# MiloszKrajewski/K4os.Compression.LZ4

Measured on NVIDIA H100. Metric: GB/s uncompressed (encode+decode) on batched 64KiB blocks @1/2/4/8 GPU vs CPU ref, higher is better.
Workload: dtype u8

## Files before the change

### k4os/compression/lz4_b200/csrc/encode_chain.cuh

```cuda
#pragma once
#include "common.cuh"
#include "encode_generic.cuh"
#include "encode_tile.cuh"

namespace k4 {

struct ChainState {
    uint32_t table[4096];
    uint32_t currentOffset;
    uint32_t dictSize;
    uint32_t reserved[2];
};
static_assert(sizeof(ChainState) == 16400, "K4LZ4_CHAIN_STATE_BYTES");

#ifndef K4_ENC_CHAIN_WARPS
#define K4_ENC_CHAIN_WARPS 32
#endif
constexpr int ENC_CHAIN_WARPS = K4_ENC_CHAIN_WARPS;

__device__ int encode_chain_warp(const uint8_t* __restrict__ src, const uint32_t n, const uint32_t P,
                                 uint8_t* __restrict__ dst, const int cap, ChainState* st) {
    const int lane = lane_id();
    uint32_t* const table = st->table;
    uint32_t startIndex = __ldcg(&st->currentOffset), dsz = __ldcg(&st->dictSize);
    if (startIndex + n > 0x80000000u) {
        const uint32_t delta = startIndex - 65536u;
        for (int i = lane; i < 4096; i += 32) {
            const uint32_t t = __ldcg(table + i);
            __stcg(table + i, t < delta ? 0u : t - delta);
        }
        startIndex = 65536u;
        if (dsz > 65536u) dsz = 65536u;
    }
    if (n > (uint32_t)MAX_INPUT_SIZE) {
        if (lane == 0) { __stcg(&st->currentOffset, startIndex); __stcg(&st->dictSize, dsz); }
        __syncwarp();
        return 0;
    }
    const uint32_t d = dsz < P ? dsz : P;
    const bool dictSmall = d < 65536u && d < startIndex;
    const uint32_t prefixIdxLimit = startIndex - d;
    if (lane == 0) { __stcg(&st->currentOffset, startIndex + n); __stcg(&st->dictSize, d + n); }
    auto accept = [&](uint32_t idx, uint32_t cur) {
        return idx < cur && !(dictSmall && idx < prefixIdxLimit) && !(idx + (uint32_t)MAX_DISTANCE < cur);
    };
#define RD32(p) ldg_u32u(src + (int)(p))
#define RD8(p) ((uint32_t)__ldg(src + (int)(p)))
#define HASH(p) hash5(ldg_u64u(src + (p)), 12)
    const int64_t olimit = cap;
    uint32_t ip = 0, anchor = 0, op = 0;

    if (n >= (uint32_t)MINLENGTH) {
        const uint32_t mfl1 = n - MFLIMIT + 1, mlim = n - LASTLITERALS;
        if (lane == 0) __stcg(table + HASH(0), startIndex);
        __syncwarp();
        ip = 1;
        bool post = false;
        uint32_t q0 = 0;
        uint32_t base = 1;
        for (;;) {
            uint32_t h2 = 0xFFFFFFFFu;
            if (post) h2 = HASH(ip - 2);
            const bool isPost = post && lane == 0;
            const uint32_t q = q0 + (uint32_t)lane - (post ? 1u : 0u);
            const uint32_t pos = isPost ? ip : base + probe_advance(q);
            const bool valid = isPost || (base + probe_advance(q + 1) <= mfl1);
            const uint64_t v64 = valid ? ldg_u64u(src + pos) : 0ull;
            const uint32_t v = (uint32_t)v64;
            const uint32_t h = valid ? hash5(v64, 12) : (0x10000u + (uint32_t)lane);
            uint32_t cand = valid ? __ldcg(table + h) : 0u;
            if (h == h2) cand = startIndex + ip - 2;
            const unsigned peers = __match_any_sync(FULL, h);
            const unsigned earlier = peers & ((1u << lane) - 1u);
            const int fromLane = earlier ? 31 - __clz(earlier) : lane;
            const uint32_t fwdPos = __shfl_sync(FULL, pos, fromLane);
            if (earlier) cand = startIndex + fwdPos;
            const uint32_t cur = startIndex + pos;
            bool hit = false;
            if (valid && accept(cand, cur)) hit = RD32(cand - startIndex) == v;
            const unsigned hits = __ballot_sync(FULL, hit);
            const unsigned ends = __ballot_sync(FULL, !valid);
            const int f = hits ? __ffs(hits) - 1 : 32;
            const int e = ends ? __ffs(ends) - 1 : 32;
            {
                const int last = e < f ? e - 1 : f;
                const unsigned upto = (last >= 31) ? 0xffffffffu : ((1u << (last + 1)) - 1u);
                const unsigned later = peers & ~((2u << lane) - 1u) & upto;
                const bool doStore = valid && ((1u << lane) & upto) && !(lane < 31 ? later : 0u);
                if (post) {
                    const unsigned same2 = __ballot_sync(FULL, valid && h == h2) & upto;
                    if (lane == 0 && !same2) __stcg(table + h2, startIndex + ip - 2);
                }
                if (doStore) __stcg(table + h, cur);
                __syncwarp();
            }
            if (e < f) break;
            if (f == 32) {
                if (post) { post = false; base = ip + 1; q0 = 31; }
                else q0 += 32;
                continue;
            }
            const bool zeroLit = post && f == 0;
            int m = (int)(__shfl_sync(FULL, cand, f) - startIndex);
            ip = __shfl_sync(FULL, pos, f);
            const uint32_t a0h = ip + MINMATCH;
            const int b0h = m + MINMATCH;
            uint32_t x1 = 0u;
            {
                const uint32_t a = a0h + 4u * lane;
                if (lane < 8 && (int)mlim - (int)a > 0) x1 = RD32(a) ^ RD32(b0h + 4 * lane);
            }
            uint32_t caught = 0;
            if (!zeroLit) {
                for (int width = 8;; width = 32) {
                    const bool part = lane < width;
                    const bool ok = !part || ((ip > anchor + lane) && (m - lane > -(int)d) &&
                                              (RD8(ip - 1 - lane) == RD8(m - 1 - lane)));
                    const unsigned bad = __ballot_sync(FULL, !ok);
                    const int c = bad ? __ffs(bad) - 1 : width;
                    ip -= c; m -= c; caught += (uint32_t)c;
                    if (bad) break;
                }
            }
            const uint32_t lit = ip - anchor;
            if (!zeroLit && (int64_t)op + 1 + lit + 8 + lit / 255 > olimit) return 0;
            uint32_t mc = caught;
            {
                uint32_t a0 = a0h;
                int b0 = b0h;
                for (int width = 8;; width = 32) {
                    const uint32_t a = a0 + 4u * lane;
                    const int bb = b0 + 4 * lane;
                    const bool part = lane < width;
                    const int room = (int)mlim - (int)a;
                    const uint32_t x = width == 8 ? x1 : ((part && room > 0) ? (RD32(a) ^ RD32(bb)) : 0u);
                    int eq = x ? ((__ffs(x) - 1) >> 3) : 4;
                    if (eq > room) eq = room < 0 ? 0 : room;
                    if (!part) eq = 4;
                    const unsigned stop = __ballot_sync(FULL, eq < 4);
                    if (stop) {
                        const int s = __ffs(stop) - 1;
                        mc += 4u * s + (uint32_t)__shfl_sync(FULL, eq, s);
                        break;
                    }
                    mc += 4u * width; a0 += 4u * width; b0 += 4 * width;
                }
            }
            const uint32_t hdr = run_header_size(lit);
            const uint32_t afterOff = op + hdr + lit + 2;
            if ((int64_t)afterOff + 6 + (mc + 240) / 255 > olimit) return 0;
            {
                const uint32_t mlTok = mc >= 15 ? 15u : mc;
                const uint32_t off = (uint32_t)((int)ip - m);
                if (lane == 0) {
                    if (lit >= 15) {
                        uint32_t o = op, rest = lit - 15;
                        dst[o++] = (uint8_t)(0xF0 | mlTok);
                        for (; rest >= 255; rest -= 255) dst[o++] = 255;
                        dst[o] = (uint8_t)rest;
                    } else dst[op] = (uint8_t)((lit << 4) | mlTok);
                    dst[afterOff - 2] = (uint8_t)off;
                    dst[afterOff - 1] = (uint8_t)(off >> 8);
                }
                for (uint32_t i = lane; i < lit; i += 32) dst[op + hdr + i] = (uint8_t)RD8(anchor + i);
                op = afterOff;
                if (mc >= 15) {
                    const uint32_t rest = mc - 15, nff = rest / 255;
                    for (uint32_t i = lane; i < nff; i += 32) dst[op + i] = 0xFF;
                    if (lane == 0) dst[op + nff] = (uint8_t)(rest % 255);
                    op += nff + 1;
                }
            }
            ip += mc + MINMATCH;
            anchor = ip;
            if (ip >= mfl1) break;
            post = true; q0 = 0; base = ip + 1;
        }
    }
    {
        const uint32_t run = n - anchor;
        if ((int64_t)op + run + 1 + (run + 255 - 15) / 255 > olimit) return 0;
        const uint32_t hdr = run_header_size(run);
        if (lane == 0) write_run_header(dst, op, run);
        op += hdr;
        for (uint32_t i = lane; i < run; i += 32) dst[op + i] = (uint8_t)RD8(anchor + i);
        op += run;
        return (int)op;
    }
#undef RD32
#undef RD8
#undef HASH
}

__global__ void __launch_bounds__(32, ENC_CHAIN_WARPS)
encode_chain_kernel(const uint8_t* __restrict__ srcBase, const int64_t* __restrict__ srcOff,
                    const int32_t* __restrict__ srcLen, const int32_t* __restrict__ prefixLen,
                    uint8_t* __restrict__ dstBase, const int64_t* __restrict__ dstOff,
                    const int32_t* __restrict__ dstCap, uint8_t* __restrict__ stateBase,
                    const int64_t* __restrict__ stateOff, int32_t* __restrict__ outLen, int nBlocks, int level,
                    uint32_t* __restrict__ nextBlock) {
    const int lane = lane_id();
    for (;;) {
        int b = 0;
        if (lane == 0) b = (int)atomicAdd(nextBlock, 1u);
        b = __shfl_sync(FULL, b, 0);
        if (b >= nBlocks) return;
        const int n = srcLen[b];
        if (n <= 0) { if (lane == 0) outLen[b] = 0; continue; }
        if (level >= 3) { if (lane == 0) outLen[b] = -2; continue; }
        const int P = prefixLen[b];
        uint8_t* const sp = stateBase + stateOff[b];
        if (P < 0 || (reinterpret_cast<uintptr_t>(sp) & 15)) { if (lane == 0) outLen[b] = -1; continue; }
        const int r = encode_chain_warp(srcBase + srcOff[b], (uint32_t)n, (uint32_t)P, dstBase + dstOff[b],
                                        dstCap[b], reinterpret_cast<ChainState*>(sp));
        if (lane == 0) {
            outLen[b] = r <= 0 ? -1 : r;
            atomicAdd(&g_encode_stats[3], 1ull);
        }
        __syncwarp();
    }
}

}
```

### k4os/compression/lz4_b200/csrc/encode_tile.cuh

```cuda
#pragma once
#include "common.cuh"
#include "encode_generic.cuh"

namespace k4 {


__device__ __forceinline__ uint32_t lds_u32u(const uint8_t* p) {
    const uintptr_t a = reinterpret_cast<uintptr_t>(p);
    const uint32_t* w = reinterpret_cast<const uint32_t*>(a & ~uintptr_t(3));
    return __funnelshift_r(w[0], w[1], (uint32_t)(a & 3) * 8);
}

#ifndef K4_ENC_OVL
#define K4_ENC_OVL 1
#endif
#ifndef K4_ENC_PF
#define K4_ENC_PF 0
#endif
#ifndef K4_ENC_WIN
#define K4_ENC_WIN 16
#endif
#ifndef K4_ENC_SPEC
#define K4_ENC_SPEC 1
#endif
static_assert(K4_ENC_WIN >= 0 && K4_ENC_WIN <= 32, "K4_ENC_WIN: lanes of a run's first batch, 1..32 (0 = 32)");
__device__ __forceinline__ void prefetch_l1(const void* p) { asm volatile("prefetch.global.L1 [%0];" :: "l"(p)); }

__device__ __forceinline__ uint32_t probe_advance(uint32_t q) {
    if (q <= 64u) return q;
    if (q == 0) return 0;
    const uint32_t c = 63u + q, k = c >> 6;
    return 1u + 32u * k * (k - 1u) + (c - 64u * k) * k;
}

template <bool STAGED, bool HARD = true, bool GTAB = false, int TAGMODE = (K4_ENC_TAGS ? 1 : 0), int WIN = 32>
__device__ int encode_spec_warp(const uint8_t* __restrict__ src, const uint8_t* sin, const uint32_t n,
                                uint8_t* __restrict__ dst, const int cap, const int hardCap, uint16_t* table) {
    const int lane = lane_id();
    const int64_t hard = hardCap;
#define RD32(p) (STAGED ? lds_u32u(sin + (p)) : ldg_u32u(src + (p)))
#ifndef K4_ENC_GTAB_L1
#define K4_ENC_GTAB_L1 0
#endif
#define TGET(h) ((GTAB && !K4_ENC_GTAB_L1) ? (uint32_t)__ldcg(table + (h)) : (uint32_t)table[(h)])
    constexpr bool TAGS = TAGMODE != 0;
    constexpr uint32_t TAG_SHIFT = TAGMODE == 2 ? 3u : 11u, TAG_MASK = TAGMODE == 2 ? 0xFFFFu : 0xFFu;
    uint8_t* const tags = reinterpret_cast<uint8_t*>(table) + ENC_TABLE_BYTES;
    uint32_t* const table32 = reinterpret_cast<uint32_t*>(table);
    auto tagGet = [&](uint32_t h) -> uint32_t {
        return (GTAB && !K4_ENC_GTAB_L1) ? (uint32_t)__ldcg(tags + h) : (uint32_t)tags[h];
    };
    auto slotPut = [&](uint32_t h, uint32_t pos, uint32_t tg) {
        if (TAGMODE == 2) {
            if (GTAB) __stcg(table32 + h, pos | (tg << 16)); else table32[h] = pos | (tg << 16);
        } else {
            if (GTAB && !K4_ENC_GTAB_L1) __stcg(table + h, (uint16_t)pos); else table[h] = (uint16_t)pos;
            if (TAGS) { if (GTAB && !K4_ENC_GTAB_L1) __stcg(tags + h, (uint8_t)tg); else tags[h] = (uint8_t)tg; }
        }
    };
#define RD8(p) (STAGED ? (uint32_t)sin[(p)] : (uint32_t)__ldg(src + (p)))
    {
        const uint32_t t0 = (TAGS && n >= 4) ? (((RD32(0) * 2654435761u) >> TAG_SHIFT) & TAG_MASK) : 0u;
        const uint32_t fillT = TAGMODE == 2 ? (t0 << 16) : 0u;
        uint4* t = reinterpret_cast<uint4*>(table);
        constexpr int TBYTES = TAGMODE == 2 ? 2 * ENC_TABLE_BYTES : ENC_TABLE_BYTES;
        for (int i = lane; i < TBYTES / 16; i += 32) {
            if (GTAB) __stcg(t + i, make_uint4(fillT, fillT, fillT, fillT)); else t[i] = make_uint4(fillT, fillT, fillT, fillT);
        }
        if (TAGMODE == 1 || TAGMODE == 3) {
            const uint32_t b4 = t0 * 0x01010101u;
            uint4* g = reinterpret_cast<uint4*>(tags);
            for (int i = lane; i < (ENC_TABLE_BYTES / 2) / 16; i += 32) {
                if (GTAB) __stcg(g + i, make_uint4(b4, b4, b4, b4)); else g[i] = make_uint4(b4, b4, b4, b4);
            }
        }
        __syncwarp();
    }
    const bool limited = !(cap >= max_output_size((int)n));
    const int64_t olimit = cap;
    uint32_t ip = 0, anchor = 0, op = 0;

    if (n >= (uint32_t)MINLENGTH) {
        const uint32_t mfl1 = n - MFLIMIT + 1, mlim = n - LASTLITERALS;
        if (lane == 0) { const uint32_t p0 = RD32(0) * 2654435761u; slotPut(p0 >> 19, 0u, (p0 >> TAG_SHIFT) & TAG_MASK); }
        __syncwarp();
        ip = 1;
        bool post = false;
        uint32_t q0 = 0;
        uint32_t base = 1;
        constexpr uint32_t WIN0 = (WIN <= 0 || WIN > 32) ? 32u : (uint32_t)WIN;
        constexpr bool NARROW = WIN0 < 32u;
        uint32_t width = WIN0;
        for (;;) {
            uint32_t h2 = 0xFFFFFFFFu, tag2 = 0;
            if (post) { const uint32_t p2 = RD32(ip - 2) * 2654435761u; h2 = p2 >> 19; tag2 = (p2 >> TAG_SHIFT) & TAG_MASK; }
            const bool isPost = post && lane == 0;
            const uint32_t q = q0 + (uint32_t)lane - (post ? 1u : 0u);
            const uint32_t pos = isPost ? ip : base + probe_advance(q);
            const bool inWin = !NARROW || (uint32_t)lane < width;
            const bool valid = inWin && (isPost || (base + probe_advance(q + 1) <= mfl1));
            const uint32_t v = valid ? RD32(pos) : 0u;
            const uint32_t prod = v * 2654435761u;
            const uint32_t h = valid ? prod >> 19 : (0x10000u + (uint32_t)lane);
            const uint32_t tg = (prod >> TAG_SHIFT) & TAG_MASK;
            uint32_t cand = 0u, ctag = tg;
            bool lazyPos = false;
            if (TAGMODE == 2) {
                const uint32_t e32 = valid ? ((GTAB && !K4_ENC_GTAB_L1) ? __ldcg(table32 + h) : table32[h]) : 0xFFFF0000u;
                cand = e32 & 0xFFFFu; ctag = e32 >> 16;
                if (!valid) ctag = 0x10000u;
            } else if (TAGMODE == 3) {
                ctag = valid ? tagGet(h) : 0x100u;
                lazyPos = true;
            } else {
                cand = valid ? TGET(h) : 0u;
                if (TAGMODE == 1) ctag = valid ? tagGet(h) : 0x100u;
            }
            if (h == h2) { cand = ip - 2; ctag = TAGS ? tag2 : tg; lazyPos = false; }
            const unsigned peers = __match_any_sync(FULL, h);
            const unsigned earlier = peers & ((1u << lane) - 1u);
            const int fromLane = earlier ? 31 - __clz(earlier) : lane;
            const uint32_t fwdPos = __shfl_sync(FULL, pos, fromLane);
            const uint32_t fwdTag = __shfl_sync(FULL, tg, fromLane);
            if (earlier) { cand = fwdPos; ctag = TAGS ? fwdTag : tg; lazyPos = false; }
            constexpr bool SPEC = K4_ENC_SPEC && TAGMODE == 2 && K4_ENC_OVL;
            bool hit = false;
            if (!SPEC && valid && ctag == tg) {
                if (TAGMODE == 3 && lazyPos) cand = TGET(h);
                hit = RD32(cand) == v;
                if (TAGS && !STAGED && (K4_ENC_PF & 1)) {
                    prefetch_l1(src + (cand + 32u < n ? cand + 32u : n - 1u));
                    if (cand >= 8u) prefetch_l1(src + cand - 8u);
                }
            }
            if (!STAGED && (K4_ENC_PF & 2) && lane == 0) prefetch_l1(src + (pos + 384u < n ? pos + 384u : n - 1u));
            const unsigned ends = __ballot_sync(FULL, inWin && !valid);
            const int e = ends ? __ffs(ends) - 1 : 32;
            int f = 32;
            uint32_t sm = 0u, sip = 0u, sx1 = 0u;
            bool sok = true;
            if (SPEC) {
                for (unsigned agree = __ballot_sync(FULL, valid && ctag == tg); agree; agree &= agree - 1u) {
                    const int c = __ffs(agree) - 1;
                    if (e < c) break;
                    sm = __shfl_sync(FULL, cand, c);
                    sip = __shfl_sync(FULL, pos, c);
                    const uint32_t vc = __shfl_sync(FULL, v, c);
                    bool same = true;
                    sx1 = 0u; sok = true;
                    if (lane < 8) {
                        const uint32_t a = sip + MINMATCH + 4u * lane;
                        if ((int)mlim - (int)a > 0) sx1 = RD32(a) ^ RD32(sm + MINMATCH + 4u * lane);
                        sok = (sip > anchor + lane) && (sm > (uint32_t)lane) && (RD8(sip - 1 - lane) == RD8(sm - 1 - lane));
                    } else if (lane == 8) {
                        same = RD32(sm) == vc;
                    }
                    if (__all_sync(FULL, same)) { f = c; break; }
                }
            } else {
                const unsigned hits = __ballot_sync(FULL, hit);
                f = hits ? __ffs(hits) - 1 : 32;
            }
            if (e < f) break;
            {
                const unsigned upto = (f >= 31) ? 0xffffffffu : ((2u << f) - 1u);
                const unsigned later = peers & ~((2u << lane) - 1u) & upto;
                const bool doStore = valid && ((1u << lane) & upto) && !(lane < 31 ? later : 0u);
                if (post) {
                    const unsigned same2 = __ballot_sync(FULL, valid && h == h2) & upto;
                    if (lane == 0 && !same2) {
                        slotPut(h2, ip - 2, tag2);
                    }
                }
                if (doStore) slotPut(h, pos, tg);
                __syncwarp();
            }
            if (f == 32) {
                const uint32_t w = NARROW ? width : 32u;
                if (post) { post = false; base = ip + 1; q0 = w - 1; }
                else q0 += w;
                width = 32;
                continue;
            }
            const bool zeroLit = post && f == 0;
            uint32_t m = SPEC ? sm : __shfl_sync(FULL, cand, f);
            ip = SPEC ? sip : __shfl_sync(FULL, pos, f);
            const uint32_t a0h = ip + MINMATCH, b0h = m + MINMATCH;
            uint32_t x1 = sx1;
            if (K4_ENC_OVL && !SPEC) {
                const uint32_t a = a0h + 4u * lane;
                if (lane < 8 && (int)mlim - (int)a > 0) x1 = RD32(a) ^ RD32(b0h + 4u * lane);
            }
            uint32_t caught = 0;
            if (!zeroLit) {
                for (int width = 8;; width = 32) {
                    const bool part = lane < width;
                    const bool ok = (SPEC && width == 8) ? sok
                                  : (!part || ((ip > anchor + lane) && (m > (uint32_t)lane) &&
                                               (RD8(ip - 1 - lane) == RD8(m - 1 - lane))));
                    const unsigned bad = __ballot_sync(FULL, !ok);
                    const int c = bad ? __ffs(bad) - 1 : width;
                    ip -= c; m -= c; caught += (uint32_t)c;
                    if (bad) break;
                }
            }
            const uint32_t lit = ip - anchor;
            if (!zeroLit && limited && (int64_t)op + 1 + lit + 8 + lit / 255 > olimit) return 0;
            uint32_t mc = caught;
            {
                uint32_t a0 = a0h, b0 = b0h;
                for (int width = 8;; width = 32) {
                    const uint32_t a = a0 + 4u * lane, bb = b0 + 4u * lane;
                    const bool part = lane < width;
                    const int room = (int)mlim - (int)a;
                    const uint32_t x = (K4_ENC_OVL && width == 8) ? x1 : ((part && room > 0) ? (RD32(a) ^ RD32(bb)) : 0u);
                    int eq = x ? ((__ffs(x) - 1) >> 3) : 4;
                    if (eq > room) eq = room < 0 ? 0 : room;
                    if (!part) eq = 4;
                    const unsigned stop = __ballot_sync(FULL, eq < 4);
                    if (stop) {
                        const int s = __ffs(stop) - 1;
                        mc += 4u * s + (uint32_t)__shfl_sync(FULL, eq, s);
                        break;
                    }
                    mc += 4u * width; a0 += 4u * width; b0 += 4u * width;
                }
            }
            const uint32_t hdr = run_header_size(lit);
            const uint32_t afterOff = op + hdr + lit + 2;
            if (limited && (int64_t)afterOff + 6 + (mc + 240) / 255 > olimit) return 0;
            if (HARD && (int64_t)afterOff + (mc >= 15 ? (mc - 15) / 255 + 1 : 0) > hard) return 0;
            {
                const uint32_t mlTok = mc >= 15 ? 15u : mc;
                if (lane == 0) {
                    if (lit >= 15) {
                        uint32_t o = op, rest = lit - 15;
                        dst[o++] = (uint8_t)(0xF0 | mlTok);
                        for (; rest >= 255; rest -= 255) dst[o++] = 255;
                        dst[o] = (uint8_t)rest;
                    } else dst[op] = (uint8_t)((lit << 4) | mlTok);
                    dst[afterOff - 2] = (uint8_t)(ip - m);
                    dst[afterOff - 1] = (uint8_t)((ip - m) >> 8);
                }
                for (uint32_t i = lane; i < lit; i += 32) dst[op + hdr + i] = RD8(anchor + i);
                op = afterOff;
                if (mc >= 15) {
                    const uint32_t rest = mc - 15, nff = rest / 255;
                    for (uint32_t i = lane; i < nff; i += 32) dst[op + i] = 0xFF;
                    if (lane == 0) dst[op + nff] = (uint8_t)(rest % 255);
                    op += nff + 1;
                }
            }
            ip += mc + MINMATCH;
            anchor = ip;
            if (ip >= mfl1) break;
            post = true; q0 = 0; base = ip + 1; width = WIN0;
        }
    }
    {
        const uint32_t run = n - anchor;
        if (limited && (int64_t)op + run + 1 + (run + 255 - 15) / 255 > olimit) return 0;
        const uint32_t hdr = run_header_size(run);
        if (HARD && (int64_t)op + hdr + run > hard) return 0;
        if (lane == 0) write_run_header(dst, op, run);
        op += hdr;
        for (uint32_t i = lane; i < run; i += 32) dst[op + i] = RD8(anchor + i);
        op += run;
        return (int)op;
    }
#undef RD32
#undef TGET
#undef RD8
}

__device__ unsigned long long g_encode_stats[4];

template <bool GTAB>
__device__ __forceinline__ void encode_persistent_warp(
        const uint8_t* __restrict__ srcBase, const int64_t* __restrict__ srcOff,
        const int32_t* __restrict__ srcLen, uint8_t* __restrict__ dstBase,
        const int64_t* __restrict__ dstOff, const int32_t* __restrict__ dstCap,
        int32_t* __restrict__ outLen, const int nBlocks, int level,
        uint32_t* __restrict__ nextBlock, uint16_t* const table, const int reserve) {
    const int lane = lane_id();
    const bool enforce32 = (level & ENC_FLAG_X32) != 0;
    level &= 0xFF;
    for (;;) {
        int b = 0;
        if (lane == 0) {
            if (GTAB && (int)*(volatile uint32_t*)nextBlock >= nBlocks - reserve) b = nBlocks;
            else b = (int)atomicAdd(nextBlock, 1u);
        }
        b = __shfl_sync(FULL, b, 0);
        if (b >= nBlocks) return;
        const int n_ = srcLen[b];
        const uint8_t* __restrict__ src = srcBase + srcOff[b];
        uint8_t* __restrict__ dst = dstBase + dstOff[b];
        const int cap = dstCap[b];
        if (n_ <= 0) { if (lane == 0) outLen[b] = 0; continue; }
        if (level >= 3) { if (lane == 0) outLen[b] = -2; continue; }
        int r;
        if (n_ >= LIMIT_64K) r = encode_block_warp(src, n_, dst, cap, 0x7fffffff, table, enforce32);
        else r = encode_spec_warp<false, false, GTAB, GTAB ? ENC_GTAG : (K4_ENC_TAGS ? 1 : 0), K4_ENC_WIN>(src, nullptr, (uint32_t)n_, dst, cap, 0x7fffffff, table);
        if (lane == 0) {
            outLen[b] = r <= 0 ? -1 : r;
            atomicAdd(&g_encode_stats[n_ >= LIMIT_64K ? 2 : (GTAB ? 1 : 0)], 1ull);
        }
        __syncwarp();
    }
}

__global__ void __launch_bounds__(32)
encode_spec_kernel(const uint8_t* __restrict__ srcBase, const int64_t* __restrict__ srcOff,
                   const int32_t* __restrict__ srcLen, uint8_t* __restrict__ dstBase,
                   const int64_t* __restrict__ dstOff, const int32_t* __restrict__ dstCap,
                   int32_t* __restrict__ outLen, int nBlocks, int level, uint32_t* __restrict__ nextBlock) {
    extern __shared__ __align__(128) uint8_t smem_encs[];
    encode_persistent_warp<false>(srcBase, srcOff, srcLen, dstBase, dstOff, dstCap, outLen, nBlocks, level,
                                  nextBlock, reinterpret_cast<uint16_t*>(smem_encs), 0);
}

__global__ void __launch_bounds__(32)
encode_spec_gtab_kernel(const uint8_t* __restrict__ srcBase, const int64_t* __restrict__ srcOff,
                        const int32_t* __restrict__ srcLen, uint8_t* __restrict__ dstBase,
                        const int64_t* __restrict__ dstOff, const int32_t* __restrict__ dstCap,
                        int32_t* __restrict__ outLen, int nBlocks, int level, uint32_t* __restrict__ nextBlock,
                        uint8_t* __restrict__ gtab, int reserve) {
    encode_persistent_warp<true>(srcBase, srcOff, srcLen, dstBase, dstOff, dstCap, outLen, nBlocks, level, nextBlock,
                                 reinterpret_cast<uint16_t*>(gtab + (size_t)blockIdx.x * ENC_GSLOT_BYTES), reserve);
}

}
```

Baseline: 51.62.

## Batch LZ4 sequence emission per warp with lane-parallel scan-based writes

Instead of writing each sequence's token, literals, offset and match-length bytes as soon as it is found (lane 0 writes headers, the warp copies literals), the encoder records up to 32 sequences, one per lane, and flushes them together. The flush uses a warp prefix sum to compute output offsets, so each lane writes its own sequence and copies short literals with word loads, while long literal runs are copied cooperatively by the whole warp. This removes serial per-sequence store work from the match-finding loop, at the cost of extra registers, divergent per-lane byte stores and deferred writes whose error and early-return paths must stay consistent.

After: 52.48 (median of 6 runs). 1.7% higher.

```diff
diff --git a/k4os/compression/lz4_b200/csrc/encode_chain.cuh b/k4os/compression/lz4_b200/csrc/encode_chain.cuh
--- a/k4os/compression/lz4_b200/csrc/encode_chain.cuh
+++ b/k4os/compression/lz4_b200/csrc/encode_chain.cuh
@@ -49,6 +49,7 @@
 #define HASH(p) hash5(ldg_u64u(src + (p)), 12)
     const int64_t olimit = cap;
     uint32_t ip = 0, anchor = 0, op = 0;
+    SeqGroup grp;
 
     if (n >= (uint32_t)MINLENGTH) {
         const uint32_t mfl1 = n - MFLIMIT + 1, mlim = n - LASTLITERALS;
@@ -149,30 +150,11 @@
             const uint32_t hdr = run_header_size(lit);
             const uint32_t afterOff = op + hdr + lit + 2;
             if ((int64_t)afterOff + 6 + (mc + 240) / 255 > olimit) return 0;
-            {
-                const uint32_t mlTok = mc >= 15 ? 15u : mc;
-                const uint32_t off = (uint32_t)((int)ip - m);
-                if (lane == 0) {
-                    if (lit >= 15) {
-                        uint32_t o = op, rest = lit - 15;
-                        dst[o++] = (uint8_t)(0xF0 | mlTok);
-                        for (; rest >= 255; rest -= 255) dst[o++] = 255;
-                        dst[o] = (uint8_t)rest;
-                    } else dst[op] = (uint8_t)((lit << 4) | mlTok);
-                    dst[afterOff - 2] = (uint8_t)off;
-                    dst[afterOff - 1] = (uint8_t)(off >> 8);
-                }
-                for (uint32_t i = lane; i < lit; i += 32) dst[op + hdr + i] = (uint8_t)RD8(anchor + i);
-                op = afterOff;
-                if (mc >= 15) {
-                    const uint32_t rest = mc - 15, nff = rest / 255;
-                    for (uint32_t i = lane; i < nff; i += 32) dst[op + i] = 0xFF;
-                    if (lane == 0) dst[op + nff] = (uint8_t)(rest % 255);
-                    op += nff + 1;
-                }
-            }
+            seq_record(grp, ip, mc, (uint32_t)((int)ip - m));
+            op = afterOff + (mc >= 15 ? (mc - 15) / 255 + 1 : 0);
             ip += mc + MINMATCH;
             anchor = ip;
+            if (grp.n == 32) seq_flush(grp, src, dst, anchor, op);
             if (ip >= mfl1) break;
             post = true; q0 = 0; base = ip + 1;
         }
@@ -181,6 +163,7 @@
         const uint32_t run = n - anchor;
         if ((int64_t)op + run + 1 + (run + 255 - 15) / 255 > olimit) return 0;
         const uint32_t hdr = run_header_size(run);
+        if (grp.n) seq_flush(grp, src, dst, anchor, op);
         if (lane == 0) write_run_header(dst, op, run);
         op += hdr;
         for (uint32_t i = lane; i < run; i += 32) dst[op + i] = (uint8_t)RD8(anchor + i);
diff --git a/k4os/compression/lz4_b200/csrc/encode_tile.cuh b/k4os/compression/lz4_b200/csrc/encode_tile.cuh
--- a/k4os/compression/lz4_b200/csrc/encode_tile.cuh
+++ b/k4os/compression/lz4_b200/csrc/encode_tile.cuh
@@ -31,6 +31,75 @@
     if (q == 0) return 0;
     const uint32_t c = 63u + q, k = c >> 6;
     return 1u + 32u * k * (k - 1u) + (c - 64u * k) * k;
+}
+
+struct SeqGroup {
+    uint32_t ip = 0, mc = 0, off = 0;
+    uint32_t anchor = 0, op = 0;
+    int n = 0;
+};
+
+__device__ __forceinline__ void seq_record(SeqGroup& g, uint32_t ip, uint32_t mc, uint32_t off) {
+    if (lane_id() == g.n) { g.ip = ip; g.mc = mc; g.off = off; }
+    ++g.n;
+}
+
+__device__ __forceinline__ void seq_flush(SeqGroup& g, const uint8_t* __restrict__ src, uint8_t* __restrict__ dst,
+                                          uint32_t anchor, uint32_t op) {
+    constexpr uint32_t SHORT = 32;
+    const int lane = lane_id();
+    const bool act = lane < g.n;
+    const uint32_t mc = g.mc;
+    const uint32_t prevEnd = __shfl_up_sync(FULL, g.ip + mc + MINMATCH, 1);
+    const uint32_t a = lane == 0 ? g.anchor : prevEnd;
+    const uint32_t lit = act ? g.ip - a : 0u;
+    const uint32_t hdr = run_header_size(lit);
+    const uint32_t size = act ? hdr + lit + 2 + (mc >= 15 ? (mc - 15) / 255 + 1 : 0) : 0u;
+    uint32_t incl = size;
+#pragma unroll
+    for (int d = 1; d < 32; d <<= 1) {
+        const uint32_t t = __shfl_up_sync(FULL, incl, d);
+        if (lane >= d) incl += t;
+    }
+    const uint32_t o = g.op + incl - size;
+    if (act) {
+        const uint32_t mlTok = mc >= 15 ? 15u : mc;
+        uint32_t p = o;
+        if (lit >= 15) {
+            dst[p++] = (uint8_t)(0xF0 | mlTok);
+            uint32_t rest = lit - 15;
+            for (; rest >= 255; rest -= 255) dst[p++] = 255;
+            dst[p++] = (uint8_t)rest;
+        } else dst[p++] = (uint8_t)((lit << 4) | mlTok);
+        if (lit - 1u < SHORT) {
+            const uint8_t* s = src + a;
+            const uint32_t mis = (uint32_t)(reinterpret_cast<uintptr_t>(s) & 3);
+            const uint32_t* w = reinterpret_cast<const uint32_t*>(s - mis);
+            uint8_t* d = dst + p - mis;
+#pragma unroll 2
+            for (uint32_t i = 0; i < lit + mis; i += 4) {
+                const uint32_t v = __ldg(w + i / 4);
+#pragma unroll
+                for (uint32_t b = 0; b < 4; b++)
+                    if (i + b >= mis && i + b < lit + mis) d[i + b] = (uint8_t)(v >> (8 * b));
+            }
+        }
+        p += lit;
+        dst[p] = (uint8_t)g.off;
+        dst[p + 1] = (uint8_t)(g.off >> 8);
+        if (mc >= 15) {
+            p += 2;
+            uint32_t rest = mc - 15;
+            for (; rest >= 255; rest -= 255) dst[p++] = 255;
+            dst[p] = (uint8_t)rest;
+        }
+    }
+    for (unsigned longs = __ballot_sync(FULL, lit > SHORT); longs; longs &= longs - 1) {
+        const int k = __ffs(longs) - 1;
+        const uint32_t la = __shfl_sync(FULL, a, k), ll = __shfl_sync(FULL, lit, k), lo = __shfl_sync(FULL, o + hdr, k);
+        for (uint32_t i = lane; i < ll; i += 32) dst[lo + i] = __ldg(src + la + i);
+    }
+    g.n = 0; g.anchor = anchor; g.op = op;
 }
 
 template <bool STAGED, bool HARD = true, bool GTAB = false, int TAGMODE = (K4_ENC_TAGS ? 1 : 0), int WIN = 32>
@@ -79,6 +148,7 @@
     const bool limited = !(cap >= max_output_size((int)n));
     const int64_t olimit = cap;
     uint32_t ip = 0, anchor = 0, op = 0;
+    SeqGroup grp;
 
     if (n >= (uint32_t)MINLENGTH) {
         const uint32_t mfl1 = n - MFLIMIT + 1, mlim = n - LASTLITERALS;
@@ -230,29 +300,11 @@
             const uint32_t afterOff = op + hdr + lit + 2;
             if (limited && (int64_t)afterOff + 6 + (mc + 240) / 255 > olimit) return 0;
             if (HARD && (int64_t)afterOff + (mc >= 15 ? (mc - 15) / 255 + 1 : 0) > hard) return 0;
-            {
-                const uint32_t mlTok = mc >= 15 ? 15u : mc;
-                if (lane == 0) {
-                    if (lit >= 15) {
-                        uint32_t o = op, rest = lit - 15;
-                        dst[o++] = (uint8_t)(0xF0 | mlTok);
-                        for (; rest >= 255; rest -= 255) dst[o++] = 255;
-                        dst[o] = (uint8_t)rest;
-                    } else dst[op] = (uint8_t)((lit << 4) | mlTok);
-                    dst[afterOff - 2] = (uint8_t)(ip - m);
-                    dst[afterOff - 1] = (uint8_t)((ip - m) >> 8);
-                }
-                for (uint32_t i = lane; i < lit; i += 32) dst[op + hdr + i] = RD8(anchor + i);
-                op = afterOff;
-                if (mc >= 15) {
-                    const uint32_t rest = mc - 15, nff = rest / 255;
-                    for (uint32_t i = lane; i < nff; i += 32) dst[op + i] = 0xFF;
-                    if (lane == 0) dst[op + nff] = (uint8_t)(rest % 255);
-                    op += nff + 1;
-                }
-            }
+            seq_record(grp, ip, mc, ip - m);
+            op = afterOff + (mc >= 15 ? (mc - 15) / 255 + 1 : 0);
             ip += mc + MINMATCH;
             anchor = ip;
+            if (grp.n == 32) seq_flush(grp, src, dst, anchor, op);
             if (ip >= mfl1) break;
             post = true; q0 = 0; base = ip + 1; width = WIN0;
         }
@@ -262,6 +314,7 @@
         if (limited && (int64_t)op + run + 1 + (run + 255 - 15) / 255 > olimit) return 0;
         const uint32_t hdr = run_header_size(run);
         if (HARD && (int64_t)op + hdr + run > hard) return 0;
+        if (grp.n) seq_flush(grp, src, dst, anchor, op);
         if (lane == 0) write_run_header(dst, op, run);
         op += hdr;
         for (uint32_t i = lane; i < run; i += 32) dst[op + i] = RD8(anchor + i);
```
